# real-stanford/semantic-abstraction

Measured on AMD Instinct MI355X. Metric: scenes/sec (relevancy+3D-UNet infer), 480x480x16-label x128^3, higher is better.
Workload: dtype f16 (MFMA operands, fp32 accumulate; UNet hi/lo-split = fp32-equivalent); 1 GPU; end-to-end relevancy->fusion->OVSSC per scene: 480x480 RGB-D, 16 labels, ViT-B/16, 'ours' saliency config (2448 tile forwards), 128^3 voxels, 80000 input points; scene-sharded; arch=ViT-B/16, unet_precision=exact, tile_chunk_streams=1, scenes_per_gpu=26, parallelism=scene-shard x1, mode=throughput

## Files before the change

include/semabs.h:

```cpp
#ifndef SEMABS_H
#define SEMABS_H
#include <stdint.h>
#ifdef __cplusplus
extern "C" {
#endif

#define SEMABS_OK 0
#define SEMABS_EINVAL (-1)
#define SEMABS_EHIP (-2)

const char* semabs_last_error(void);
int semabs_abi_version(void);
int semabs_stream_create_cumask(const unsigned int* mask, int n_words, void** stream);
int semabs_stream_destroy(void* stream);
int semabs_stream_cu_count(void* stream, int* cus);

int semabs_fill_u32(void* p, long long nbytes, unsigned int value, void* stream);
int semabs_replicate(const void* src, void* dst, long long nbytes, int reps, void* stream);
int semabs_copy2d(const void* src, long long src_pitch_bytes, void* dst, long long dst_pitch_bytes, long long width_bytes, long long rows, void* stream);
int semabs_poison_empty(const long long* n_in, float* logits, long long n_logits, int* labels, long long n_labels, void* stream);
int semabs_device_info(char* name , int name_len, int* cu_count , long long* hbm_bytes );


int semabs_pointcloud(const float* depth, int H, int W, const double* params, int has_pose, float* xyz,
// ... 84 lines not shown

int semabs_point_mlp(const float* xyz, const float* feat, const float* w1, const float* b1, const float* w2, const float* b2,
                     const float* w3, const float* b3, float* out, int P, long N, int hidden, int cout, void* stream);
int semabs_point_mlp_fma(const float* xyz, const float* feat, const float* w1, const float* b1, const float* w2, const float* b2,
                         const float* w3, const float* b3, float* out, int P, long N, int hidden, int cout, void* stream);
int semabs_scatter_mean(const long long* flat, const float* feat, int* head, int* next, void* vol, int P, long N, int C,
                        long nvox, int vol_f32, void* stream);
int semabs_scatter_mean_stats(const long long* flat, const float* feat, int* head, int* next, void* vol, int P, long N, int C,
                              long nvox, int vol_f32, double* out_sums, void* stream);
int semabs_scatter_mean_sparse(const long long* flat, const float* feat, int* head, int* next, void* vol, unsigned int* occ, int P, long N, int C, long nvox,
                               int vol_f32, double* out_sums, void* stream);
int semabs_gn_stats(const void* x, double* sums, int B, long nvox, int C, int G, int x_f32, void* stream);
int semabs_gn_finalize(const double* sums, const float* gamma, const float* beta, float* scale, float* shift, int B, int C,
                       int G, long nvox, float eps, void* stream);
int semabs_conv3d(const void* x, const void* w_hi, const void* w_lo, void* y, const float* gn_scale, const float* gn_shift,
                  const float* bias, const void* resid, int B, int D0, int D1, int D2, int Cin, int Cout, int ksize, int relu,
                  int act_f32, void* stream);
int semabs_conv3d_stats(const void* x, const void* w_hi, const void* w_lo, void* y, const float* gn_scale, const float* gn_shift,
                        const float* bias, const void* resid, int B, int D0, int D1, int D2, int Cin, int Cout, int ksize, int relu,
                        int act_f32, double* out_sums, int out_groups, void* stream);
int semabs_conv3d_sparse_stats(const void* x, const unsigned int* occ, const void* w_hi, const void* w_lo, void* y, const float* gn_scale, const float* gn_shift,
                               const float* bias, const void* resid, int B, int D0, int D1, int D2, int Cin, int Cout, int ksize, int relu, int act_f32,
                               double* out_sums, int out_groups, void* stream);
int semabs_convtranspose3d(const void* x, const void* w_hi, const void* w_lo, const long* class_off , void* y,
                           const float* bias, const void* skip, int B, int D0, int D1, int D2, int Cin, int Cout, int act_f32,
                           void* stream);
int semabs_convtranspose3d_stats(const void* x, const void* w_hi, const void* w_lo, const long* class_off, void* y, const float* bias,
                                 const void* skip, int B, int D0, int D1, int D2, int Cin, int Cout, int act_f32, double* out_sums,
                                 int out_groups, void* stream);
int semabs_maxpool3d(const void* x, void* y, int B, int D0, int D1, int D2, int C, int act_f32, void* stream);
int semabs_decoder(const void* vol, const float* query, const float* off3, const float* sc3, const int* shape3, const float* w1,
                   const float* b1, const float* w2, const float* b2, int concat_xyz, int P, long M, long q_stride_p, int vol_f32,
                   float* out, const int* qgrid3, const float* final_w, const float* final_b, void* stream);

int semabs_vool_head(const void* vol_t, const void* vol_r, const float* query, const float* params, const float* rel,
                     const float* off3, const float* sc3, const int* shape3, float temperature, int P, long M, int vol_f32,
                     float* out, void* stream);


int semabs_lamb_step(const long long* chunks, int n_chunks, const long long* ptrs, int n_tensors, double lr, double beta1,
                     double beta2, double eps, double weight_decay, int adam, double* norms, float* stats, void* stream);


int semabs_conv3d_gather(const void* x, const void* w_hi, const void* w_lo, void* y, const float* in_scale, const float* in_shift, int B,
                         int I0, int I1, int I2, int M0, int M1, int M2, int in_stride, int Cin, int Cout, int ntaps, const signed char* taps,
                         int act_f32, void* stream);
// ... 83 lines not shown
```

semantic-abstraction_amd/_lib.py:

```python
from __future__ import annotations

import ctypes as C
import os

import torch

_HERE = os.path.dirname(os.path.abspath(__file__))
LIB_PATH = os.path.join(_HERE, "lib", "libsemabs_hip.so")
if os.environ.get("SEMABS_LIB_PATH"):
    LIB_PATH = os.environ["SEMABS_LIB_PATH"]
elif os.environ.get("SEMABS_TUNE_LIB") == "1":
    LIB_PATH = os.path.join(_HERE, "lib", "libsemabs_hip_tune.so")

_lib = None

P = C.c_void_p
I = C.c_int
L = C.c_long
F = C.c_float
D = C.c_double

SIGNATURES = {
    "semabs_abi_version": [],
    "semabs_stream_create_cumask": [P, I, P],
# ... 35 lines not shown
    "semabs_rows_gather": [P, P, L, I, L, L, P],
    "semabs_eot_rows_gather": [P, P, P, I, I, I, P],
    "semabs_quickgelu": [P, P, L, I, P],
    "semabs_quickgelu_grad": [P, P, L, P],
    "semabs_logit_grad": [P, P, I, I, I, P, P, P, I, P],
    "semabs_ln_bwd": [P, P, P, P, P, P, L, I, I, L, F, I, P],
    "semabs_gelu_bwd": [P, P, P, L, I, I, I, P],
    "semabs_rollout": [P, P, P, P, P, I, I, I, I, I, L, L, P],
    "semabs_gather_text": [P, P, P, P, I, I, I, P],
    "semabs_attention_bwd": [P, P, P, P, P, P, P, P, P, I, I, I, I, I, I, P],
    "semabs_seq_rescale": [P, P, P, L, L, P],
    "semabs_rollout_step": [P, P, L, P],
    "semabs_text_finish": [P, P, I, I, I, P],
    "semabs_point_mlp": [P, P, P, P, P, P, P, P, P, I, L, I, I, P],
    "semabs_point_mlp_fma": [P, P, P, P, P, P, P, P, P, I, L, I, I, P],
    "semabs_scatter_mean": [P, P, P, P, P, I, L, I, L, I, P],
    "semabs_scatter_mean_stats": [P, P, P, P, P, I, L, I, L, I, P, P],
    "semabs_scatter_mean_sparse": [P, P, P, P, P, P, I, L, I, L, I, P, P],
    "semabs_gn_stats": [P, P, I, L, I, I, I, P],
    "semabs_gn_finalize": [P, P, P, P, P, I, I, I, L, F, P],
    "semabs_conv3d": [P, P, P, P, P, P, P, P, I, I, I, I, I, I, I, I, I, P],
    "semabs_conv3d_stats": [P, P, P, P, P, P, P, P, I, I, I, I, I, I, I, I, I, P, I, P],
    "semabs_conv3d_sparse_stats": [P, P, P, P, P, P, P, P, P, I, I, I, I, I, I, I, I, I, P, I, P],
    "semabs_convtranspose3d": [P, P, P, C.POINTER(C.c_long), P, P, P, I, I, I, I, I, I, I, P],
    "semabs_convtranspose3d_stats": [P, P, P, C.POINTER(C.c_long), P, P, P, I, I, I, I, I, I, I, P, I, P],
    "semabs_maxpool3d": [P, P, I, I, I, I, I, I, P],
    "semabs_vool_head": [P, P, P, P, P, C.POINTER(F), C.POINTER(F), C.POINTER(I), F, I, L, I, P, P],
    "semabs_lamb_step": [P, I, P, I, D, D, D, D, D, I, P, P, P],
    "semabs_decoder": [P, P, C.POINTER(F), C.POINTER(F), C.POINTER(I), P, P, P, P, I, I, L, L, I, P, C.POINTER(I), P, P, P],
    "semabs_conv3d_gather": [P, P, P, P, P, P, I, I, I, I, I, I, I, I, I, I, I, C.c_char_p, I, P],
    "semabs_wgrad": [P, P, P, P, P, I, I, I, I, I, I, I, I, I, I, I, C.c_char_p, I, P],
    "semabs_wgrad_mfma": [P, P, P, P, P, P, P, I, I, I, I, I, I, I, I, I, I, I, C.c_char_p, I, P, L, P],
    "semabs_wgrad_conv3": [P, P, P, P, P, P, I, I, I, I, I, I, I, P, L, P],
    "semabs_wgrad_conv3_supported": [I, I, I, I, I, L, C.POINTER(I)],
    "semabs_conv3d_gnbwd_supported": [I, I, I, I, I, I, I, I, C.POINTER(I)],
    "semabs_conv3d_gnbwd": [P, P, P, P, P, P, P, P, P, P, I, P, I, P, I, I, I, I, I, I, I, P],
    "semabs_wgrad_conv3_gn_supported": [I, I, I, I, I, I, L, C.POINTER(I)],
    "semabs_wgrad_conv3_gn": [P, P, P, P, I, P, P, P, P, P, P, I, I, I, I, I, I, P, L, P],
    "semabs_chan_reduce": [P, P, P, P, P, I, L, I, I, P],
    "semabs_gn_meanrstd": [P, P, P, I, I, L, F, P],
    "semabs_gn_bwd_coef": [P, P, P, P, P, P, P, I, I, I, L, P],
    "semabs_gn_bwd_apply": [P, P, P, P, P, P, P, P, P, P, I, L, I, I, P],
    "semabs_ew": [P, P, P, L, I, F, P, P],
    "semabs_ew_scaled": [P, P, P, P, L, I, F, P, P],
    "semabs_grad_scale": [P, L, P, P, I, P, P, I, P],
    "semabs_maxpool3d_bwd": [P, P, P, I, I, I, I, I, P],
# ... 116 lines not shown
```

semantic-abstraction_amd/csrc/unet.hip:

```cpp
#include "semabs_common.h"

__device__ __forceinline__ int xcd_remap(int vb, int nb) {
    const int q = nb >> 3, r = nb & 7, x = vb & 7, k = vb >> 3;
    return (x < r ? x * (q + 1) : r * (q + 1) + (x - r) * q) + k;
}
__device__ __forceinline__ int xcd_persistent_tile(int vb, int G, int it, int total) {
    if (G & 7) { const long t = (long)it * G + vb; return t < total ? (int)t : -1; }
    const int x = vb & 7, j = vb >> 3, g8 = G >> 3;
    const int q = total >> 3, r = total & 7;
    const int lo = x < r ? x * (q + 1) : r * (q + 1) + (x - r) * q, cnt = q + (x < r ? 1 : 0);
    const long o = (long)it * g8 + j;
    return o < cnt ? lo + (int)o : -1;
}


template <int HID, int COUT>
__global__ __launch_bounds__(256, 2) void k_point_mlp(const float* __restrict__ xyz, const float* __restrict__ feat,
                                                   const float* __restrict__ w1, const float* __restrict__ b1,
                                                   const float* __restrict__ w2, const float* __restrict__ b2,
                                                   const float* __restrict__ w3, const float* __restrict__ b3,
                                                   float* __restrict__ out, int P, long N) {
    extern __shared__ __attribute__((aligned(16))) char smem[];
    float* sw2 = reinterpret_cast<float*>(smem);
    float* sw3 = sw2 + HID * HID;
// ... 384 lines not shown
#define CONV16_ABL(c) false
#endif
struct ConvArgs {
    const void* x; void* y; const f16* w_hi; const f16* w_lo;
    const float* gn_scale; const float* gn_shift; const float* bias; const void* resid;
    int B, I0, I1, I2;
    int O0, O1, O2;
    int M0, M1, M2;
    int os, op0, op1, op2;
    int Cin, Cout, Kp;
    int ntaps; int relu;
    int is;
    int ksplit;
    signed char td0[28], td1[28], td2[28];
    double* stats;
    int ablate;
    long long* trace;
    const f16* wp_hi; const f16* wp_lo;
    int ncls; long cls_off[8];
    const float* gnb_coef = nullptr; const float* gnb_mean = nullptr; const float* gnb_rstd = nullptr; int gnb_G = 0, gnb_relu = 0;
    unsigned int* gnb_bits = nullptr;
    const unsigned int* occ = nullptr;
    const float* gnb_add = nullptr;
};

template <bool F32>
__device__ __forceinline__ void load8(const void* base, long idx, float (&v)[8]) {
    if (F32) {
        const float4* p = reinterpret_cast<const float4*>(reinterpret_cast<const float*>(base) + idx);
        float4 a = p[0], b = p[1];
        v[0] = a.x; v[1] = a.y; v[2] = a.z; v[3] = a.w; v[4] = b.x; v[5] = b.y; v[6] = b.z; v[7] = b.w;
    } else {
        f16x8 h = *reinterpret_cast<const f16x8*>(reinterpret_cast<const f16*>(base) + idx);
#pragma unroll
        for (int j = 0; j < 8; ++j) v[j] = (float)h[j];
    }
}

template <int NW, bool F32, bool CIN16, bool LDSW = false, bool CLS = false>
__global__ __launch_bounds__(256) void k_conv(ConvArgs a) {
    const int ccls = CLS ? (int)blockIdx.z : 0;
    const int cp0 = CLS ? ccls >> 2 : 0, cp1 = CLS ? (ccls >> 1) & 1 : 0, cp2 = CLS ? ccls & 1 : 0;
    const int k_ntaps = CLS ? (cp0 + 1) * (cp1 + 1) * (cp2 + 1) : a.ntaps;
    const int k_Kp = CLS ? k_ntaps * a.Cin : a.Kp;
    const int k_op0 = CLS ? cp0 : a.op0, k_op1 = CLS ? cp1 : a.op1, k_op2 = CLS ? cp2 : a.op2;
    const long k_woff = CLS ? a.cls_off[ccls] : 0;
// ... 185 lines not shown
#pragma unroll
                for (int j = 0; j < 4; ++j) o[j] = o[j] > 0.f ? o[j] : 0.01f * o[j];
            }
            if (F32) {
                *reinterpret_cast<float4*>(reinterpret_cast<float*>(a.y) + oidx) = make_float4(o[0], o[1], o[2], o[3]);
            } else {
                f16x4 h; h[0] = (f16)o[0]; h[1] = (f16)o[1]; h[2] = (f16)o[2]; h[3] = (f16)o[3];
                *reinterpret_cast<f16x4*>(reinterpret_cast<f16*>(a.y) + oidx) = h;
            }
        }
    }
}

#define C16_T1 8
#define C16_T2 16
#define C16_H1 (C16_T1 + 2)
#define C16_H2 (C16_T2 + 2)

__device__ __forceinline__ void conv_absmax_commit(unsigned int* bits, float m) {
#pragma unroll
    for (int o = 1; o < 64; o <<= 1) m = fmaxf(m, __shfl_xor(m, o, 64));
    if ((threadIdx.x & 63) == 0) atomicMax(bits, __float_as_uint(m));
}
template <bool F32, int C16_T0, bool GNB = false, bool SPARSE = false>
__global__ __launch_bounds__(512) void k_conv16_lds(ConvArgs a) {
    constexpr int C16_H0 = C16_T0 + 2, C16_HALO = C16_H0 * C16_H1 * C16_H2;
    constexpr int PLANE = (C16_HALO * 8 + 127) / 128 * 128;
    constexpr int BUF_EL = PLANE * 2 * (F32 ? 2 : 1);
    extern __shared__ __attribute__((aligned(16))) char smem[];
    const int tid = threadIdx.x, lane = tid & 63;
    const int wid = __builtin_amdgcn_readfirstlane(tid >> 6);
    const int vl = lane & 15, kg = lane >> 4;
    const int n2 = a.I2 / C16_T2, n1 = a.I1 / C16_T1, n0 = a.I0 / C16_T0;
    const int per_vol = n0 * n1 * n2, total = a.B * per_vol;
    const bool has_gn = a.gn_scale != nullptr;
    const bool producer = wid >= 4;
    const int ptid = tid - 256;
    float* const s_gnb = reinterpret_cast<float*>(smem + (size_t)BUF_EL * 2 * 2);
    if (GNB) {
        for (int e = tid; e < a.B * 16; e += 512) {
            const int b = e >> 4, c = e & 15, g = c / (16 / a.gnb_G);
            const float mu = a.gnb_mean[b * a.gnb_G + g], rs = a.gnb_rstd[b * a.gnb_G + g];
            const float* k = a.gnb_coef + (long)e * 3;
            s_gnb[b * 48 + c] = k[0]; s_gnb[b * 48 + 16 + c] = -rs * k[2]; s_gnb[b * 48 + 32 + c] = mu * rs * k[2] - k[1];
        }
    }
    float amax = 0.f;

    auto produce = [&](int brick, int buf) {
        const int b = brick / per_vol; int t = brick - b * per_vol;
        const int t2 = t % n2; t /= n2;
        const int t1 = t % n1; const int t0 = t / n1;
        const int z0 = t0 * C16_T0, y0 = t1 * C16_T1, x0 = t2 * C16_T2;
        f16* s_hi = reinterpret_cast<f16*>(smem) + buf * BUF_EL;
        f16* s_lo = s_hi + PLANE * 2;
        const int hsel = (ptid >> 3) & 1;
        const int vsub = (ptid & 7) + ((ptid >> 4) << 3);
        float gs[8], gh[8];
        if (has_gn) {
            const float4* ps = reinterpret_cast<const float4*>(a.gn_scale + b * 16 + hsel * 8);
            const float4* pt = reinterpret_cast<const float4*>(a.gn_shift + b * 16 + hsel * 8);
            const float4 s0 = ps[0], s1 = ps[1], h0 = pt[0], h1 = pt[1];
            gs[0] = s0.x; gs[1] = s0.y; gs[2] = s0.z; gs[3] = s0.w; gs[4] = s1.x; gs[5] = s1.y; gs[6] = s1.z; gs[7] = s1.w;
            gh[0] = h0.x; gh[1] = h0.y; gh[2] = h0.z; gh[3] = h0.w; gh[4] = h1.x; gh[5] = h1.y; gh[6] = h1.z; gh[7] = h1.w;
        } else {
#pragma unroll
            for (int j = 0; j < 8; ++j) { gs[j] = 1.f; gh[j] = 0.f; }
        }
        constexpr int NT = (C16_HALO + 127) / 128;
// ... 69 lines not shown
                if (F32) wl[dy][st] = *reinterpret_cast<const f16x8*>(a.w_lo + widx);
            }
    };
    const int half = kg & 1, tsel = kg >> 1;
    f32x4 bias4 = f32x4{0.f, 0.f, 0.f, 0.f};
    if (a.bias) bias4 = *reinterpret_cast<const f32x4*>(a.bias + 4 * kg);
    const float relu_floor = a.relu ? 0.f : -__builtin_inff();
    double st[4] = {0.0, 0.0, 0.0, 0.0};
    int st_b = -1;
    auto flush_stats = [&]() {
        if (st_b >= 0) {
#pragma unroll
            for (int j = 0; j < 4; ++j) {
                double v = st[j];
#pragma unroll
                for (int m = 1; m < 16; m <<= 1) v += __shfl_xor(v, m, 64);
                if (vl == 0) atomicAdd(a.stats + ((long)st_b * 8 + 2 * kg + (j >> 1)) * 2 + (j & 1), v);
                st[j] = 0.0;
            }
        }
    };
    constexpr int ROWS_PER_WAVE = C16_T0 * 2;

    auto consume = [&](int brick, int buf) {
        const int b = brick / per_vol; int t = brick - b * per_vol;
        const int t2 = t % n2; t /= n2;
        const int t1 = t % n1; const int t0 = t / n1;
        const int z0 = t0 * C16_T0, y0 = t1 * C16_T1, x0 = t2 * C16_T2;
        const f16* s_hi = reinterpret_cast<const f16*>(smem) + buf * BUF_EL;
        const f16* s_lo = s_hi + PLANE * 2;
        const size_t vol_off = (size_t)b * a.I0 * a.I1 * a.I2 * 16;
        if (a.stats && b != st_b) { flush_stats(); st_b = b; }
        constexpr int MR = 8;
        int tapoff[5];
#pragma unroll
        for (int st = 0; st < 5; ++st) {
            const int qa = 2 * st, qb = 2 * st + 1 < 9 ? 2 * st + 1 : 2 * st;
            const int q = tsel ? qb : qa;
            tapoff[st] = ((q / 3) * C16_H1 * C16_H2 + (q % 3)) * 8;
        }
#pragma unroll 1
        for (int pr = 0; pr < ROWS_PER_WAVE / MR; ++pr) {
            const int zl = (wid * ROWS_PER_WAVE + pr * MR) >> 3;
            const int fbase = half * PLANE + (zl * C16_H1 * C16_H2 + vl) * 8;
            f32x4 acc[MR];
#pragma unroll
            for (int mi = 0; mi < MR; ++mi) acc[mi] = f32x4{0.f, 0.f, 0.f, 0.f};
            unsigned ooff[MR];
            f32x4 res[MR];
#pragma unroll
            for (int mi = 0; mi < MR; ++mi) {
                ooff[mi] = (unsigned)((((z0 + zl) * a.I1 + (y0 + mi)) * a.I2 + (x0 + vl)) * 16 + 4 * kg);
                res[mi] = f32x4{0.f, 0.f, 0.f, 0.f};
            }
            if (a.resid) {
// ... 24 lines not shown
                    const int i = st * 10 + ri, slot = i % 3, rho = RHO[ri];
                    bool first = true;
#pragma unroll
                    for (int kind = 0; kind < (F32 ? 3 : 1); ++kind) {
#pragma unroll
                        for (int dy = 0; dy < 3; ++dy) {
                            const int r = rho - dy;
                            if (r < 0 || r >= MR) continue;
                            acc[r] = __builtin_amdgcn_mfma_f32_16x16x32_f16(kind == 1 ? wl[dy][st] : wh[dy][st], kind == 2 ? xl[slot] : xh[slot], acc[r], 0, 0, 0);
                            if (first) {
                                first = false;
                                if (i + 2 < 50) request(i + 2, (i + 2) % 3);
                                __builtin_amdgcn_sched_barrier(0);
                            }
                        }
                    }
                    __builtin_amdgcn_sched_barrier(0);
                }
            }
#ifdef SEMABS_TUNING
            if (a.ablate == 4) { if (acc[0][0] != 1234.5f) continue; }
#endif
            float ps[4] = {0.f, 0.f, 0.f, 0.f};
            f32x4 cA, cB, cC;
            f32x4 ad[MR];
            if (GNB && a.gnb_add) {
                ad[0] = *reinterpret_cast<const f32x4*>(a.gnb_add + vol_off + ooff[0]);
                ad[1] = *reinterpret_cast<const f32x4*>(a.gnb_add + vol_off + ooff[1]);
            }
            if (GNB) {
                cA = *reinterpret_cast<const f32x4*>(s_gnb + b * 48 + 4 * kg); cB = *reinterpret_cast<const f32x4*>(s_gnb + b * 48 + 16 + 4 * kg);
                cC = *reinterpret_cast<const f32x4*>(s_gnb + b * 48 + 32 + 4 * kg);
            }
#pragma unroll
            for (int mi = 0; mi < MR; ++mi) {
                float o[4];
                if (GNB) {
                    if (a.gnb_add && mi + 2 < MR) { ad[mi + 2] = *reinterpret_cast<const f32x4*>(a.gnb_add + vol_off + ooff[mi + 2]); __builtin_amdgcn_sched_barrier(0); }
#pragma unroll
                    for (int e = 0; e < 4; ++e) {
                        o[e] = acc[mi][e] * cA[e] + (res[mi][e] * cB[e] + cC[e]);
                        if (a.gnb_add) o[e] += ad[mi][e];
                        if (a.gnb_relu) o[e] = res[mi][e] > 0.f ? o[e] : 0.f;
                        amax = fmaxf(amax, fabsf(o[e]));
                    }
                } else {
#pragma unroll
                for (int e = 0; e < 4; ++e) o[e] = fmaxf(acc[mi][e] + bias4[e] + res[mi][e], relu_floor);
                }
                if (!F32) {
#pragma unroll
                    for (int e = 0; e < 4; ++e) o[e] = (float)(f16)o[e];
                }
                ps[0] += o[0] + o[1]; ps[1] += o[0] * o[0] + o[1] * o[1];
                ps[2] += o[2] + o[3]; ps[3] += o[2] * o[2] + o[3] * o[3];
                if (F32) {
                    *reinterpret_cast<float4*>(reinterpret_cast<float*>(a.y) + vol_off + ooff[mi]) = make_float4(o[0], o[1], o[2], o[3]);
                } else {
                    f16x4 h; h[0] = (f16)o[0]; h[1] = (f16)o[1]; h[2] = (f16)o[2]; h[3] = (f16)o[3];
                    *reinterpret_cast<f16x4*>(reinterpret_cast<f16*>(a.y) + vol_off + ooff[mi]) = h;
                }
            }
            if (a.stats) {
#pragma unroll
                for (int j = 0; j < 4; ++j) st[j] += (double)ps[j];
            }
        }
    };

    auto lds_barrier = [&]() { asm volatile("s_waitcnt lgkmcnt(0)\n\ts_barrier" ::: "memory"); };
    auto brick_of = [&](int it) { return xcd_persistent_tile((int)blockIdx.x, (int)gridDim.x, it, total); };
    if (producer) {
        int it = 0, brick = brick_of(0);
        if (brick >= 0) produce(brick, 0);
        lds_barrier();
        int buf = 0;
        for (; brick >= 0; buf ^= 1) {
            const int next = brick_of(++it);
            if (next >= 0 && !CONV16_ABL(a.ablate == 2 || a.ablate >= 4)) produce(next, buf ^ 1);
            lds_barrier();
            brick = next;
        }
    } else {
        load_weights();
        lds_barrier();
        int buf = 0, it = 0;
        for (int brick = brick_of(0); brick >= 0; brick = brick_of(++it), buf ^= 1) {
            if (!CONV16_ABL(a.ablate == 1)) consume(brick, buf);
            lds_barrier();
        }
        if (a.stats) flush_stats();
        if (GNB && a.gnb_bits) conv_absmax_commit(a.gnb_bits, amax);
    }
}

#define SEMABS_CONV_GENERIC 256
#define SEMABS_CONV_PACKED 512
#ifdef SEMABS_TUNING
static int g_conv16_ablate = 0;
static long long* g_conv_trace = nullptr;
static int g_brick_persist = 0;
static int g_convt_no_line = 0;
extern "C" int semabs_conv_tune(int key, long long value) {
    if (key == 0) g_conv16_ablate = (int)value & 7;
    else if (key == 1) g_conv_trace = reinterpret_cast<long long*>(value);
    else if (key == 2) g_brick_persist = (int)value;
    else if (key == 3) g_convt_no_line = (int)value;
    return SEMABS_OK;
}
#endif

static int conv16_lds_launch(const ConvArgs& a_in, int f32, hipStream_t s) {
    ConvArgs a = a_in;
#ifdef SEMABS_TUNING
    a.ablate = g_conv16_ablate;
#endif
    if (f32) {
        constexpr int T0 = 4;
        const size_t lds = (size_t)(((T0 + 2) * C16_H1 * C16_H2 * 8 + 127) / 128 * 128) * 2 * 2 * 2 * 2;
        const long total = (long)a.B * (a.I0 / T0) * (a.I1 / C16_T1) * (a.I2 / C16_T2);
        long nb = semabs_stream_cus(s); if (nb > total) nb = total;
        if (a.gnb_coef) {
            static SemabsLdsAttr attrg;
            semabs_ensure_lds(&k_conv16_lds<true, T0, true>, (int)(lds + 32 * 192), attrg);
            hipLaunchKernelGGL((k_conv16_lds<true, T0, true>), dim3((unsigned)nb), dim3(512), lds + (size_t)a.B * 192, s, a);
            SEMABS_CHECK_LAUNCH();
            return SEMABS_OK;
        }
        if (a.occ) {
            static SemabsLdsAttr attrs;
            semabs_ensure_lds(&k_conv16_lds<true, T0, false, true>, (int)lds, attrs);
            hipLaunchKernelGGL((k_conv16_lds<true, T0, false, true>), dim3((unsigned)nb), dim3(512), lds, s, a);
            SEMABS_CHECK_LAUNCH();
            return SEMABS_OK;
        }
        static SemabsLdsAttr attr;
        semabs_ensure_lds(&k_conv16_lds<true, T0>, (int)lds, attr);
        hipLaunchKernelGGL((k_conv16_lds<true, T0>), dim3((unsigned)nb), dim3(512), lds, s, a);
    } else {
        constexpr int T0 = 8;
        const size_t lds = (size_t)(((T0 + 2) * C16_H1 * C16_H2 * 8 + 127) / 128 * 128) * 2 * 2 * 2;
        const long total = (long)a.B * (a.I0 / T0) * (a.I1 / C16_T1) * (a.I2 / C16_T2);
        long nb = semabs_stream_cus(s); if (nb > total) nb = total;
        if (a.occ) {
            static SemabsLdsAttr attrs;
            semabs_ensure_lds(&k_conv16_lds<false, T0, false, true>, (int)lds, attrs);
            hipLaunchKernelGGL((k_conv16_lds<false, T0, false, true>), dim3((unsigned)nb), dim3(512), lds, s, a);
            SEMABS_CHECK_LAUNCH();
            return SEMABS_OK;
        }
        static SemabsLdsAttr attr;
        semabs_ensure_lds(&k_conv16_lds<false, T0>, (int)lds, attr);
        hipLaunchKernelGGL((k_conv16_lds<false, T0>), dim3((unsigned)nb), dim3(512), lds, s, a);
    }
    SEMABS_CHECK_LAUNCH();
    return SEMABS_OK;
}

template <bool F32, int CW, int NB, bool ONE, bool PERSIST, int TX = 16, bool GNB = false>
__global__ __launch_bounds__(512) void k_conv_brick(ConvArgs a, int total) {
    constexpr int T0 = 4, H0 = T0 + 2, HX = TX + 2, HALO = H0 * C16_H1 * HX, NTHR = 512;
    constexpr int R = TX / 4;
    constexpr int CPV = CW / 8;
    constexpr int NSTEPS = CW == 32 ? 27 : 14;
    constexpr bool EARLY = false;
    extern __shared__ __attribute__((aligned(16))) char smem[];
    constexpr int PLANE = (HALO * 8 + 127) / 128 * 128;
    f16* s_hi = reinterpret_cast<f16*>(smem);
    f16* s_lo = s_hi + PLANE * CPV;
    const int tid = threadIdx.x, lane = tid & 63;
// ... 423 lines not shown
#define CONV_NW(F_, C_) { if (nw == 4) CONV_GO(4, F_, C_); else if (nw == 2) CONV_GO(2, F_, C_); else CONV_GO(1, F_, C_); }
    if (nw == 4 && !c16) {
        if (f32) hipLaunchKernelGGL((k_conv<4, true, false, true>), grid, block, 0, s, a);
        else hipLaunchKernelGGL((k_conv<4, false, false, true>), grid, block, 0, s, a);
    }
    else if (f32) { if (c16) CONV_NW(true, true) else CONV_NW(true, false) }
    else { if (c16) CONV_NW(false, true) else CONV_NW(false, false) }
#undef CONV_NW
#undef CONV_GO
    SEMABS_CHECK_LAUNCH();
    return SEMABS_OK;
}

static int conv_common_checks(const void* x, const void* w_hi, const void* w_lo, void* y, int Cin, int Cout, int f32) {
    SEMABS_REQUIRE(x && w_hi && y, "semabs conv: null pointer");
    SEMABS_REQUIRE(!f32 || w_lo, "semabs conv: exact (fp32) mode needs the lo half of the split weights");
    SEMABS_REQUIRE(Cin == 16 || Cin % 32 == 0, "semabs conv: Cin must be 16 or a multiple of 32");
    SEMABS_REQUIRE(Cout % 16 == 0 && (Cout < 64 || Cout % 64 == 0), "semabs conv: Cout must be 16, 32 or a multiple of 64");
    return SEMABS_OK;
}

static int conv3d_impl(const void* x, const void* w_hi, const void* w_lo, void* y, const float* gn_scale, const float* gn_shift,
                       const float* bias, const void* resid, int B, int D0, int D1, int D2, int Cin, int Cout, int ksize,
                       int relu, int act_flags, double* out_sums, int out_groups, void* stream, const unsigned int* occ = nullptr) {
    if (B == 0) return SEMABS_OK;
    const int act_f32 = act_flags & 1;
    const bool bricks = !(act_flags & SEMABS_CONV_GENERIC);
    int rc = conv_common_checks(x, w_hi, w_lo, y, Cin, Cout, act_f32);
    if (rc) return rc;
    SEMABS_REQUIRE(ksize == 1 || ksize == 3, "semabs_conv3d: kernel size must be 1 or 3");
    SEMABS_REQUIRE((gn_scale == nullptr) == (gn_shift == nullptr), "semabs_conv3d: gn_scale and gn_shift go together");
    ConvArgs a;
    a.x = x; a.y = y; a.w_hi = (const f16*)w_hi; a.w_lo = (const f16*)w_lo; a.gn_scale = gn_scale; a.gn_shift = gn_shift;
    a.bias = bias; a.resid = resid; a.B = B; a.I0 = D0; a.I1 = D1; a.I2 = D2; a.O0 = D0; a.O1 = D1; a.O2 = D2;
    a.M0 = D0; a.M1 = D1; a.M2 = D2; a.os = 1; a.is = 1; a.op0 = a.op1 = a.op2 = 0; a.Cin = Cin; a.Cout = Cout; a.relu = relu;
    a.ntaps = ksize * ksize * ksize;
    a.Kp = ((a.ntaps * Cin + 31) / 32) * 32;
    a.stats = nullptr; a.ablate = 0; a.trace = nullptr; a.wp_hi = nullptr; a.wp_lo = nullptr; a.ncls = 0;
    if (act_flags & SEMABS_CONV_PACKED) {
        a.wp_hi = a.w_hi + (long)Cout * a.Kp;
        if (w_lo) a.wp_lo = a.w_lo + (long)Cout * a.Kp;
    }
    int t = 0;
    for (int kd = 0; kd < ksize; ++kd)
        for (int kh = 0; kh < ksize; ++kh)
            for (int kw = 0; kw < ksize; ++kw, ++t) { a.td0[t] = kd - ksize / 2; a.td1[t] = kh - ksize / 2; a.td2[t] = kw - ksize / 2; }
    SEMABS_REQUIRE(relu == 0 || relu == 1 || (relu == 2 && ksize == 1), "semabs_conv3d: relu must be 0, 1, or 2 (LeakyReLU, ksize 1 only)");
    SEMABS_REQUIRE(!out_sums || (out_groups > 0 && Cout % out_groups == 0), "semabs_conv3d_stats: Cout must be a multiple of out_groups");
    bool fused = false;
    if (bricks && ksize == 3 && Cin == 16 && Cout == 16 && D0 % 8 == 0 && D1 % C16_T1 == 0 && D2 % C16_T2 == 0 && (long)D0 * D1 * D2 * 16 < (1L << 31)) {
        if (out_sums && out_groups == 8) { a.stats = out_sums; fused = true; }
        a.occ = occ;
        rc = conv16_lds_launch(a, act_f32, (hipStream_t)stream);
    } else if (occ) {
        semabs_set_error("semabs_conv3d_sparse_stats: the occupancy bitmap is read by the 16 -> 16 level-0 kernel only (D0 % 8, D1 % 8, D2 % 16 == 0)");
        return SEMABS_EINVAL;
    } else if (bricks && ksize == 3 && (Cout % 32 == 0 || (Cout == 16 && Cin % 32 == 0 && D2 % C16_T2 == 0)) && (Cin == 16 || Cin % 32 == 0) && relu != 2 &&
               D0 % 4 == 0 && D1 % C16_T1 == 0 && (D2 % C16_T2 == 0 || (D2 % 8 == 0 && Cin % 32 == 0))) {
        if (out_sums && out_groups == 8 && Cout >= 32) { a.stats = out_sums; fused = true; }
        rc = conv_brick_launch(a, act_f32, (hipStream_t)stream);
    } else {
        rc = conv_launch(a, act_f32, (hipStream_t)stream);
    }
    if (rc == SEMABS_OK && out_sums && !fused) rc = semabs_gn_stats(y, out_sums, B, (long)D0 * D1 * D2, Cout, out_groups, act_f32, stream);
    return rc;
}
extern "C" int semabs_conv3d(const void* x, const void* w_hi, const void* w_lo, void* y, const float* gn_scale, const float* gn_shift,
                             const float* bias, const void* resid, int B, int D0, int D1, int D2, int Cin, int Cout, int ksize,
                             int relu, int act_f32, void* stream) {
    return conv3d_impl(x, w_hi, w_lo, y, gn_scale, gn_shift, bias, resid, B, D0, D1, D2, Cin, Cout, ksize, relu, act_f32, nullptr, 0, stream);
}
extern "C" int semabs_conv3d_stats(const void* x, const void* w_hi, const void* w_lo, void* y, const float* gn_scale, const float* gn_shift,
                                   const float* bias, const void* resid, int B, int D0, int D1, int D2, int Cin, int Cout, int ksize,
                                   int relu, int act_f32, double* out_sums, int out_groups, void* stream) {
    SEMABS_REQUIRE(out_sums, "semabs_conv3d_stats: out_sums is null");
    return conv3d_impl(x, w_hi, w_lo, y, gn_scale, gn_shift, bias, resid, B, D0, D1, D2, Cin, Cout, ksize, relu, act_f32, out_sums, out_groups, stream);
}

extern "C" int semabs_conv3d_sparse_stats(const void* x, const unsigned int* occ, const void* w_hi, const void* w_lo, void* y, const float* gn_scale, const float* gn_shift,
                                          const float* bias, const void* resid, int B, int D0, int D1, int D2, int Cin, int Cout, int ksize,
                                          int relu, int act_f32, double* out_sums, int out_groups, void* stream) {
    SEMABS_REQUIRE(out_sums && occ, "semabs_conv3d_sparse_stats: out_sums / occ is null");
    SEMABS_REQUIRE(!(act_f32 & SEMABS_CONV_GENERIC), "semabs_conv3d_sparse_stats: the generic kernel reads the whole volume");
    return conv3d_impl(x, w_hi, w_lo, y, gn_scale, gn_shift, bias, resid, B, D0, D1, D2, Cin, Cout, ksize, relu, act_f32, out_sums, out_groups, stream, occ);
}

static int conv3d_gnbwd_route(int B, int D0, int D1, int D2, int Cin, int Cout, int G, bool have_add) {
    if (B <= 0 || G <= 0) return 0;
    if (B <= 32 && Cin == 16 && Cout == 16 && D0 % 8 == 0 && D1 % C16_T1 == 0 && D2 % C16_T2 == 0 && (long)D0 * D1 * D2 * 16 < (1L << 31) && 16 % G == 0) return 1;
    if (!have_add && Cin % 32 == 0 && Cout % 32 == 0 && Cout % G == 0 && (Cout / G) % 4 == 0 && D0 % 4 == 0 && D1 % C16_T1 == 0 && D2 % C16_T2 == 0) return 2;
    return 0;
}
extern "C" int semabs_conv3d_gnbwd_supported(int B, int D0, int D1, int D2, int Cin, int Cout, int G, int have_add1, int* ok) {
    SEMABS_REQUIRE(ok, "semabs_conv3d_gnbwd_supported: null pointer");
    *ok = conv3d_gnbwd_route(B, D0, D1, D2, Cin, Cout, G, have_add1 != 0) ? 1 : 0;
    return SEMABS_OK;
}
extern "C" int semabs_conv3d_gnbwd(const void* dZ, const void* w_hi, const void* w_lo, void* dX, const float* in_scale, const float* in_shift, const void* X,
                                   const float* mean, const float* rstd, const float* coef, int G, const float* add1, int relu_mask, unsigned int* absmax_bits,
                                   int B, int D0, int D1, int D2, int Cin, int Cout, int act_flags, void* stream) {
    if (B == 0) return SEMABS_OK;
    SEMABS_REQUIRE(dZ && w_hi && w_lo && dX && X && mean && rstd && coef, "semabs_conv3d_gnbwd: null pointer");
    const int route = conv3d_gnbwd_route(B, D0, D1, D2, Cin, Cout, G, add1 != nullptr);
    SEMABS_REQUIRE((act_flags & 1) && route, "semabs_conv3d_gnbwd: exact mode and a supported shape (see semabs_conv3d_gnbwd_supported)");
    SEMABS_REQUIRE((in_scale == nullptr) == (in_shift == nullptr), "semabs_conv3d_gnbwd: in_scale and in_shift go together");
    ConvArgs a;
    a.x = dZ; a.y = dX; a.w_hi = (const f16*)w_hi; a.w_lo = (const f16*)w_lo; a.gn_scale = in_scale; a.gn_shift = in_shift;
// ... 609 lines not shown
```

semantic-abstraction_amd/unet3d.py:

```python
from __future__ import annotations

import ctypes as C
from typing import Dict, List

import numpy as np
import torch

from . import _lib


def number_of_features_per_level(init_channel_number, num_levels):
    return [init_channel_number * 2 ** k for k in range(num_levels)]



def _pack_fragments(w: torch.Tensor) -> torch.Tensor:
    cout, kp = int(w.shape[0]), int(w.shape[1])
    assert cout % 16 == 0 and kp % 32 == 0
    return w.reshape(cout // 16, 16, kp // 32, 4, 8).permute(2, 0, 3, 1, 4).contiguous().reshape(-1)


def matrix_layout(m: torch.Tensor):
    rows, k = int(m.shape[0]), int(m.shape[1])
    kp = (k + 31) // 32 * 32
# ... 71 lines not shown
    def __init__(self, weight: torch.Tensor, bias, dev):
        flat, packed, offs = convT_class_layout(weight.float())
        self._set((*_split16(flat, dev), packed, offs), weight.shape, bias.float().to(dev).contiguous())

    def _set(self, fwd, wshape, bias):
        self.w_hi, self.w_lo, self.packed, offs = fwd
        self.class_off = (C.c_long * 8)(*offs)
        self.cin, self.cout = int(wshape[0]), int(wshape[1])
        self.bias = bias

    @classmethod
    def of(cls, name, fwd, bwd, wshape, bias):
        r = cls.__new__(cls)
        r.name, r.bwd = name, bwd
        r._set(fwd, wshape, bias)
        return r


class _Rec:
    __slots__ = ("name", "x", "y", "mean", "rstd", "scale", "shift")



def gn_conv(x, conv: _Conv, relu, zeros, f32, resid=None, gn=True, in_sums=None, out_groups=0, generic=False, occ=None, rec: _Rec | None = None):
    B, D0, D1, D2, Cc = x.shape
    nvox, dev, st = D0 * D1 * D2, x.device, _lib.stream()
    scale = shift = None
    if gn:
        G, sums = conv.groups, in_sums
        if sums is None:
            sums = zeros((B, G, 2), torch.float64)
            _lib.call("semabs_gn_stats", _lib.ptr(x), _lib.ptr(sums), B, nvox, Cc, G, f32, st)
        scale = torch.empty(B, Cc, dtype=torch.float32, device=dev)
        shift = torch.empty_like(scale)
        _lib.call("semabs_gn_finalize", _lib.ptr(sums), _lib.ptr(conv.gn_w), _lib.ptr(conv.gn_b), _lib.ptr(scale), _lib.ptr(shift),
                  B, Cc, G, nvox, 1e-5, st)
        if rec is not None:
            rec.mean = torch.empty(B, G, dtype=torch.float32, device=dev)
            rec.rstd = torch.empty_like(rec.mean)
            _lib.call("semabs_gn_meanrstd", _lib.ptr(sums), _lib.ptr(rec.mean), _lib.ptr(rec.rstd), B, G, nvox * (Cc // G), 1e-5, st)
    y = torch.empty(B, D0, D1, D2, conv.cout, dtype=torch.float32 if f32 else torch.float16, device=dev)
    if rec is not None:
        rec.name, rec.x, rec.y, rec.scale, rec.shift = conv.name, x, y, scale, shift
    args = (_lib.ptr(x), _lib.ptr(conv.w_hi), _lib.ptr(conv.w_lo), _lib.ptr(y), _lib.ptr(scale), _lib.ptr(shift),
            _lib.ptr(conv.bias), _lib.ptr(resid), B, D0, D1, D2, conv.cin, conv.cout, conv.k, int(relu), f32 | (256 if generic else 0) | conv.packed)
    if not out_groups:
        assert occ is None
        _lib.call("semabs_conv3d", *args, st)
        return y, None
    out_sums = zeros((B, out_groups, 2), torch.float64)
    if occ is not None:
        _lib.call("semabs_conv3d_sparse_stats", args[0], _lib.ptr(occ), *args[1:], _lib.ptr(out_sums), out_groups, st)
    else:
        _lib.call("semabs_conv3d_stats", *args, _lib.ptr(out_sums), out_groups, st)
    return y, out_sums


def res_block(x, convs, zeros, f32, in_sums=None, occ=None, tape=None):
    r1, r2, r3 = (None,) * 3 if tape is None else (_Rec(), _Rec(), _Rec())
    out1, s1 = gn_conv(x, convs[0], True, zeros, f32, in_sums=in_sums, out_groups=convs[1].groups, occ=occ, rec=r1)
    out2, s2 = gn_conv(out1, convs[1], True, zeros, f32, in_sums=s1, out_groups=convs[2].groups, rec=r2)
    y, _ = gn_conv(out2, convs[2], True, zeros, f32, resid=out1, in_sums=s2, rec=r3)
    if tape is not None:
        tape.append(("block", r1, r2, r3))
    return y


def maxpool(x, f32):
    B, D0, D1, D2, Cc = x.shape
    y = torch.empty(B, D0 // 2, D1 // 2, D2 // 2, Cc, dtype=x.dtype, device=x.device)
    _lib.call("semabs_maxpool3d", _lib.ptr(x), _lib.ptr(y), B, D0, D1, D2, Cc, f32, _lib.stream())
    return y


def up_conv(x, skip, ct: _ConvT, zeros, f32, out_groups=0, generic=False):
    B, D0, D1, D2, _ = x.shape
    assert tuple(skip.shape) == (B, 2 * D0, 2 * D1, 2 * D2, ct.cout)
    y = torch.empty_like(skip)
    args = (_lib.ptr(x), _lib.ptr(ct.w_hi), _lib.ptr(ct.w_lo), ct.class_off, _lib.ptr(y),
            _lib.ptr(ct.bias), _lib.ptr(skip), B, D0, D1, D2, ct.cin, ct.cout, f32 | (256 if generic else 0) | ct.packed)
    if not out_groups:
        _lib.call("semabs_convtranspose3d", *args, _lib.stream())
        return y, None
    sums = zeros((B, out_groups, 2), torch.float64)
    _lib.call("semabs_convtranspose3d_stats", *args, _lib.ptr(sums), out_groups, _lib.stream())
    return y, sums


def unet_forward(x, enc, dec, final: _Conv, zeros, f32, in_sums=None, occ=None, taps=None, skip_final=False, tape=None, rows_w=None):
    feats = []
    for i, convs in enumerate(enc):
        if i > 0:
            if tape is not None:
                tape.append(("pool", x, i - 1))
            x = maxpool(x, f32)
        x = res_block(x, convs, zeros, f32, in_sums=in_sums if i == 0 else None, occ=occ if i == 0 else None, tape=tape)
        if taps is not None:
            taps[f"enc{i}"] = x
        feats.insert(0, x)
    for i, (skip, (ct, convs)) in enumerate(zip(feats[1:], dec)):
        y, sums = up_conv(x, skip, ct, zeros, f32, out_groups=convs[0].groups)
        if tape is not None:
            tape.append(("up", ct.name, x, len(enc) - 2 - i))
        x = res_block(y, convs, zeros, f32, in_sums=sums, tape=tape)
        if taps is not None:
            taps[f"dec{i}"] = x
    if skip_final:
        return x
    if tape is not None:
        tape.append(("final", x))
    if rows_w is None:
        return gn_conv(x, final, False, zeros, f32, gn=False)[0]
    B, D0, D1, D2, _ = x.shape
    y = torch.empty(B, D0, D1, D2, final.cout, dtype=torch.float32, device=x.device)
    _lib.call("semabs_linear_rows", _lib.ptr(x), final.cin, _lib.ptr(rows_w), final.cin, 1, _lib.ptr(final.bias), _lib.ptr(y),
              B * D0 * D1 * D2, final.cin, final.cout, 0, 0.0, None, None, None, None, None, None, _lib.stream())
    return y


# ... 110 lines not shown
```

Before: 8.723 scenes/s.

## Fuse 2x2x2 maxpool and next-level GroupNorm stats into encoder conv epilogue

Adds a pooling variant of the 16-channel LDS conv kernel. It computes the 2x2x2 max inside the epilogue using DPP lane swaps and an LDS staging area, writes the pooled volume, and accumulates the GroupNorm sums for the next encoder level. The aim is to remove the separate maxpool launch and its full re-read of the level output, and to feed the next res_block's first conv with precomputed stats. Shapes that do not fit the kernel fall back to separate maxpool and gn_stats calls inside the same entry point. The cost is extra LDS per block, which may lower occupancy, plus an extra join phase after each brick's barrier.

```diff
diff --git a/include/semabs.h b/include/semabs.h
--- a/include/semabs.h
+++ b/include/semabs.h
@@ -130,6 +130,9 @@
 int semabs_conv3d_sparse_stats(const void* x, const unsigned int* occ, const void* w_hi, const void* w_lo, void* y, const float* gn_scale, const float* gn_shift,
                                const float* bias, const void* resid, int B, int D0, int D1, int D2, int Cin, int Cout, int ksize, int relu, int act_f32,
                                double* out_sums, int out_groups, void* stream);
+int semabs_conv3d_pool_stats(const void* x, const void* w_hi, const void* w_lo, void* y, void* y_pool, const float* gn_scale, const float* gn_shift,
+                             const float* bias, const void* resid, int B, int D0, int D1, int D2, int Cin, int Cout, int ksize, int relu,
+                             int act_f32, double* pool_sums, int pool_groups, void* stream);
 int semabs_convtranspose3d(const void* x, const void* w_hi, const void* w_lo, const long* class_off , void* y,
                            const float* bias, const void* skip, int B, int D0, int D1, int D2, int Cin, int Cout, int act_f32,
                            void* stream);
diff --git a/semantic-abstraction_amd/_lib.py b/semantic-abstraction_amd/_lib.py
--- a/semantic-abstraction_amd/_lib.py
+++ b/semantic-abstraction_amd/_lib.py
@@ -81,6 +81,7 @@
     "semabs_conv3d": [P, P, P, P, P, P, P, P, I, I, I, I, I, I, I, I, I, P],
     "semabs_conv3d_stats": [P, P, P, P, P, P, P, P, I, I, I, I, I, I, I, I, I, P, I, P],
     "semabs_conv3d_sparse_stats": [P, P, P, P, P, P, P, P, P, I, I, I, I, I, I, I, I, I, P, I, P],
+    "semabs_conv3d_pool_stats": [P, P, P, P, P, P, P, P, P, I, I, I, I, I, I, I, I, I, P, I, P],
     "semabs_convtranspose3d": [P, P, P, C.POINTER(C.c_long), P, P, P, I, I, I, I, I, I, I, P],
     "semabs_convtranspose3d_stats": [P, P, P, C.POINTER(C.c_long), P, P, P, I, I, I, I, I, I, I, P, I, P],
     "semabs_maxpool3d": [P, P, I, I, I, I, I, I, P],
diff --git a/semantic-abstraction_amd/csrc/unet.hip b/semantic-abstraction_amd/csrc/unet.hip
--- a/semantic-abstraction_amd/csrc/unet.hip
+++ b/semantic-abstraction_amd/csrc/unet.hip
@@ -430,6 +430,7 @@
     unsigned int* gnb_bits = nullptr;
     const unsigned int* occ = nullptr;
     const float* gnb_add = nullptr;
+    void* y_pool = nullptr;
 };
 
 template <bool F32>
@@ -661,8 +662,9 @@
     for (int o = 1; o < 64; o <<= 1) m = fmaxf(m, __shfl_xor(m, o, 64));
     if ((threadIdx.x & 63) == 0) atomicMax(bits, __float_as_uint(m));
 }
-template <bool F32, int C16_T0, bool GNB = false, bool SPARSE = false>
+template <bool F32, int C16_T0, bool GNB = false, bool SPARSE = false, bool POOL = false>
 __global__ __launch_bounds__(512) void k_conv16_lds(ConvArgs a) {
+    static_assert(!(POOL && (GNB || SPARSE)), "the pooling epilogue is instantiated for the plain forward kernel only");
     constexpr int C16_H0 = C16_T0 + 2, C16_HALO = C16_H0 * C16_H1 * C16_H2;
     constexpr int PLANE = (C16_HALO * 8 + 127) / 128 * 128;
     constexpr int BUF_EL = PLANE * 2 * (F32 ? 2 : 1);
@@ -684,6 +686,7 @@
             s_gnb[b * 48 + c] = k[0]; s_gnb[b * 48 + 16 + c] = -rs * k[2]; s_gnb[b * 48 + 32 + c] = mu * rs * k[2] - k[1];
         }
     }
+    float* const s_pool = reinterpret_cast<float*>(smem + (size_t)BUF_EL * 2 * 2);
     float amax = 0.f;
 
     auto produce = [&](int brick, int buf) {
@@ -799,7 +802,7 @@
     };
     constexpr int ROWS_PER_WAVE = C16_T0 * 2;
 
-    auto consume = [&](int brick, int buf) {
+    auto consume = [&](int brick, int buf, [[maybe_unused]] int par) {
         const int b = brick / per_vol; int t = brick - b * per_vol;
         const int t2 = t % n2; t /= n2;
         const int t1 = t % n1; const int t0 = t / n1;
@@ -807,7 +810,7 @@
         const f16* s_hi = reinterpret_cast<const f16*>(smem) + buf * BUF_EL;
         const f16* s_lo = s_hi + PLANE * 2;
         const size_t vol_off = (size_t)b * a.I0 * a.I1 * a.I2 * 16;
-        if (a.stats && b != st_b) { flush_stats(); st_b = b; }
+        if (!POOL && a.stats && b != st_b) { flush_stats(); st_b = b; }
         constexpr int MR = 8;
         int tapoff[5];
 #pragma unroll
@@ -878,6 +881,7 @@
             if (a.ablate == 4) { if (acc[0][0] != 1234.5f) continue; }
 #endif
             float ps[4] = {0.f, 0.f, 0.f, 0.f};
+            [[maybe_unused]] float prow[4] = {0.f, 0.f, 0.f, 0.f};
             f32x4 cA, cB, cC;
             f32x4 ad[MR];
             if (GNB && a.gnb_add) {
@@ -910,6 +914,22 @@
                 }
                 ps[0] += o[0] + o[1]; ps[1] += o[0] * o[0] + o[1] * o[1];
                 ps[2] += o[2] + o[3]; ps[3] += o[2] * o[2] + o[3] * o[3];
+                if constexpr (POOL) {
+                    if (mi & 1) {
+                        int pl = lane;
+                        asm volatile("" : "+v"(pl));
+                        f32x4 m;
+#pragma unroll
+                        for (int e = 0; e < 4; ++e) {
+                            const float v = fmaxf(prow[e], o[e]);
+                            m[e] = fmaxf(v, __int_as_float(__builtin_amdgcn_update_dpp(0, __float_as_int(v), 0xB1, 0xF, 0xF, true)));
+                        }
+                        if (!(pl & 1)) *reinterpret_cast<f32x4*>(s_pool + (((par * C16_T0 + zl) * 4 + (mi >> 1)) * 8 + ((pl & 15) >> 1)) * 16 + 4 * (pl >> 4)) = m;
+                    } else {
+#pragma unroll
+                        for (int e = 0; e < 4; ++e) prow[e] = o[e];
+                    }
+                }
                 if (F32) {
                     *reinterpret_cast<float4*>(reinterpret_cast<float*>(a.y) + vol_off + ooff[mi]) = make_float4(o[0], o[1], o[2], o[3]);
                 } else {
@@ -917,7 +937,7 @@
                     *reinterpret_cast<f16x4*>(reinterpret_cast<f16*>(a.y) + vol_off + ooff[mi]) = h;
                 }
             }
-            if (a.stats) {
+            if (!POOL && a.stats) {
 #pragma unroll
                 for (int j = 0; j < 4; ++j) st[j] += (double)ps[j];
             }
@@ -940,12 +960,55 @@
     } else {
         load_weights();
         lds_barrier();
+        [[maybe_unused]] auto flush_pool_stats = [&]() {
+            if (st_b >= 0) {
+#pragma unroll
+                for (int j = 0; j < 4; ++j) {
+                    double v = st[j];
+#pragma unroll
+                    for (int m = 4; m < 64; m <<= 1) v += __shfl_xor(v, m, 64);
+                    if (lane < 4) atomicAdd(a.stats + ((long)st_b * 8 + 2 * lane + (j >> 1)) * 2 + (j & 1), v);
+                    st[j] = 0.0;
+                }
+            }
+        };
+        [[maybe_unused]] auto join_pool = [&](int brick, int par) {
+            const int b = brick / per_vol; int t = brick - b * per_vol;
+            const int t2 = t % n2; t /= n2;
+            const int t1 = t % n1; const int t0 = t / n1;
+            const int P1 = a.I1 >> 1, P2 = a.I2 >> 1;
+            int pl = lane;
+            asm volatile("" : "+v"(pl));
+#pragma unroll
+            for (int j = 0; j < C16_T0 / 4; ++j) {
+                const int c = wid * (C16_T0 / 4) + j, p = c >> 1, py = (c & 1) * 2 + (pl >> 5), px = (pl >> 2) & 7, ch = (pl & 3) * 4;
+                const float* s0 = s_pool + (((par * C16_T0 + 2 * p) * 4 + py) * 8 + px) * 16 + ch;
+                const f32x4 u = *reinterpret_cast<const f32x4*>(s0), v = *reinterpret_cast<const f32x4*>(s0 + 4 * 8 * 16);
+                const float m0 = fmaxf(u[0], v[0]), m1 = fmaxf(u[1], v[1]), m2 = fmaxf(u[2], v[2]), m3 = fmaxf(u[3], v[3]);
+                if (a.stats) {
+                    if (b != st_b) { flush_pool_stats(); st_b = b; }
+                    const double d0 = (double)m0, d1 = (double)m1, d2 = (double)m2, d3 = (double)m3;
+                    st[0] += d0 + d1; st[1] += d0 * d0 + d1 * d1;
+                    st[2] += d2 + d3; st[3] += d2 * d2 + d3 * d3;
+                }
+                const size_t oidx = (size_t)b * (a.I0 >> 1) * P1 * P2 * 16 +
+                                    (unsigned)((((t0 * (C16_T0 / 2) + p) * P1 + t1 * (C16_T1 / 2) + py) * P2 + t2 * (C16_T2 / 2) + px) * 16 + ch);
+                if (F32) {
+                    *reinterpret_cast<float4*>(reinterpret_cast<float*>(a.y_pool) + oidx) = make_float4(m0, m1, m2, m3);
+                } else {
+                    f16x4 h; h[0] = (f16)m0; h[1] = (f16)m1; h[2] = (f16)m2; h[3] = (f16)m3;
+                    *reinterpret_cast<f16x4*>(reinterpret_cast<f16*>(a.y_pool) + oidx) = h;
+                }
+            }
+        };
         int buf = 0, it = 0;
         for (int brick = brick_of(0); brick >= 0; brick = brick_of(++it), buf ^= 1) {
-            if (!CONV16_ABL(a.ablate == 1)) consume(brick, buf);
+            if (!CONV16_ABL(a.ablate == 1)) consume(brick, buf, it & 1);
             lds_barrier();
-        }
-        if (a.stats) flush_stats();
+            if constexpr (POOL) join_pool(brick, it & 1);
+        }
+        if (!POOL && a.stats) flush_stats();
+        if constexpr (POOL) { if (a.stats) flush_pool_stats(); }
         if (GNB && a.gnb_bits) conv_absmax_commit(a.gnb_bits, amax);
     }
 }
@@ -990,6 +1053,13 @@
             SEMABS_CHECK_LAUNCH();
             return SEMABS_OK;
         }
+        if (a.y_pool) {
+            static SemabsLdsAttr attrp;
+            semabs_ensure_lds(&k_conv16_lds<true, T0, false, false, true>, (int)(lds + 2 * T0 * 2048), attrp);
+            hipLaunchKernelGGL((k_conv16_lds<true, T0, false, false, true>), dim3((unsigned)nb), dim3(512), lds + 2 * T0 * 2048, s, a);
+            SEMABS_CHECK_LAUNCH();
+            return SEMABS_OK;
+        }
         static SemabsLdsAttr attr;
         semabs_ensure_lds(&k_conv16_lds<true, T0>, (int)lds, attr);
         hipLaunchKernelGGL((k_conv16_lds<true, T0>), dim3((unsigned)nb), dim3(512), lds, s, a);
@@ -1002,6 +1072,13 @@
             static SemabsLdsAttr attrs;
             semabs_ensure_lds(&k_conv16_lds<false, T0, false, true>, (int)lds, attrs);
             hipLaunchKernelGGL((k_conv16_lds<false, T0, false, true>), dim3((unsigned)nb), dim3(512), lds, s, a);
+            SEMABS_CHECK_LAUNCH();
+            return SEMABS_OK;
+        }
+        if (a.y_pool) {
+            static SemabsLdsAttr attrp;
+            semabs_ensure_lds(&k_conv16_lds<false, T0, false, false, true>, (int)(lds + 2 * T0 * 2048), attrp);
+            hipLaunchKernelGGL((k_conv16_lds<false, T0, false, false, true>), dim3((unsigned)nb), dim3(512), lds + 2 * T0 * 2048, s, a);
             SEMABS_CHECK_LAUNCH();
             return SEMABS_OK;
         }
@@ -1471,7 +1548,8 @@
 
 static int conv3d_impl(const void* x, const void* w_hi, const void* w_lo, void* y, const float* gn_scale, const float* gn_shift,
                        const float* bias, const void* resid, int B, int D0, int D1, int D2, int Cin, int Cout, int ksize,
-                       int relu, int act_flags, double* out_sums, int out_groups, void* stream, const unsigned int* occ = nullptr) {
+                       int relu, int act_flags, double* out_sums, int out_groups, void* stream, const unsigned int* occ = nullptr,
+                       void* y_pool = nullptr, double* pool_sums = nullptr, int pool_groups = 0, int* pooled = nullptr) {
     if (B == 0) return SEMABS_OK;
     const int act_f32 = act_flags & 1;
     const bool bricks = !(act_flags & SEMABS_CONV_GENERIC);
@@ -1500,6 +1578,10 @@
     if (bricks && ksize == 3 && Cin == 16 && Cout == 16 && D0 % 8 == 0 && D1 % C16_T1 == 0 && D2 % C16_T2 == 0 && (long)D0 * D1 * D2 * 16 < (1L << 31)) {
         if (out_sums && out_groups == 8) { a.stats = out_sums; fused = true; }
         a.occ = occ;
+        if (y_pool && !occ) {
+            a.y_pool = y_pool; *pooled = 1;
+            if (!out_sums && pool_groups == 8) { a.stats = pool_sums; *pooled = 2; }
+        }
         rc = conv16_lds_launch(a, act_f32, (hipStream_t)stream);
     } else if (occ) {
         semabs_set_error("semabs_conv3d_sparse_stats: the occupancy bitmap is read by the 16 -> 16 level-0 kernel only (D0 % 8, D1 % 8, D2 % 16 == 0)");
@@ -1532,6 +1614,21 @@
     SEMABS_REQUIRE(out_sums && occ, "semabs_conv3d_sparse_stats: out_sums / occ is null");
     SEMABS_REQUIRE(!(act_f32 & SEMABS_CONV_GENERIC), "semabs_conv3d_sparse_stats: the generic kernel reads the whole volume");
     return conv3d_impl(x, w_hi, w_lo, y, gn_scale, gn_shift, bias, resid, B, D0, D1, D2, Cin, Cout, ksize, relu, act_f32, out_sums, out_groups, stream, occ);
+}
+
+extern "C" int semabs_maxpool3d(const void* x, void* y, int B, int D0, int D1, int D2, int C, int act_f32, void* stream);
+extern "C" int semabs_conv3d_pool_stats(const void* x, const void* w_hi, const void* w_lo, void* y, void* y_pool, const float* gn_scale, const float* gn_shift,
+                                        const float* bias, const void* resid, int B, int D0, int D1, int D2, int Cin, int Cout, int ksize,
+                                        int relu, int act_f32, double* pool_sums, int pool_groups, void* stream) {
+    SEMABS_REQUIRE(y_pool && pool_sums, "semabs_conv3d_pool_stats: y_pool / pool_sums is null");
+    SEMABS_REQUIRE(D0 % 2 == 0 && D1 % 2 == 0 && D2 % 2 == 0 && Cout % 8 == 0, "semabs_conv3d_pool_stats: dims must be even, Cout % 8 == 0");
+    SEMABS_REQUIRE(pool_groups > 0 && Cout % pool_groups == 0, "semabs_conv3d_pool_stats: Cout must be a multiple of pool_groups");
+    int pooled = 0;
+    int rc = conv3d_impl(x, w_hi, w_lo, y, gn_scale, gn_shift, bias, resid, B, D0, D1, D2, Cin, Cout, ksize, relu, act_f32, nullptr, 0, stream, nullptr, y_pool,
+                         pool_sums, pool_groups, &pooled);
+    if (rc == SEMABS_OK && pooled < 1) rc = semabs_maxpool3d(y, y_pool, B, D0, D1, D2, Cout, act_f32 & 1, stream);
+    if (rc == SEMABS_OK && pooled < 2) rc = semabs_gn_stats(y_pool, pool_sums, B, (long)(D0 / 2) * (D1 / 2) * (D2 / 2), Cout, pool_groups, act_f32 & 1, stream);
+    return rc;
 }
 
 static int conv3d_gnbwd_route(int B, int D0, int D1, int D2, int Cin, int Cout, int G, bool have_add) {
diff --git a/semantic-abstraction_amd/unet3d.py b/semantic-abstraction_amd/unet3d.py
--- a/semantic-abstraction_amd/unet3d.py
+++ b/semantic-abstraction_amd/unet3d.py
@@ -117,7 +117,8 @@
 
 
 
-def gn_conv(x, conv: _Conv, relu, zeros, f32, resid=None, gn=True, in_sums=None, out_groups=0, generic=False, occ=None, rec: _Rec | None = None):
+def gn_conv(x, conv: _Conv, relu, zeros, f32, resid=None, gn=True, in_sums=None, out_groups=0, generic=False, occ=None, rec: _Rec | None = None,
+            pool_groups=0):
     B, D0, D1, D2, Cc = x.shape
     nvox, dev, st = D0 * D1 * D2, x.device, _lib.stream()
     scale = shift = None
@@ -139,6 +140,12 @@
         rec.name, rec.x, rec.y, rec.scale, rec.shift = conv.name, x, y, scale, shift
     args = (_lib.ptr(x), _lib.ptr(conv.w_hi), _lib.ptr(conv.w_lo), _lib.ptr(y), _lib.ptr(scale), _lib.ptr(shift),
             _lib.ptr(conv.bias), _lib.ptr(resid), B, D0, D1, D2, conv.cin, conv.cout, conv.k, int(relu), f32 | (256 if generic else 0) | conv.packed)
+    if pool_groups:
+        assert not out_groups and occ is None and rec is None
+        y_pool = torch.empty(B, D0 // 2, D1 // 2, D2 // 2, conv.cout, dtype=y.dtype, device=dev)
+        pool_sums = zeros((B, pool_groups, 2), torch.float64)
+        _lib.call("semabs_conv3d_pool_stats", *args[:4], _lib.ptr(y_pool), *args[4:], _lib.ptr(pool_sums), pool_groups, st)
+        return y, (y_pool, pool_sums)
     if not out_groups:
         assert occ is None
         _lib.call("semabs_conv3d", *args, st)
@@ -151,14 +158,17 @@
     return y, out_sums
 
 
-def res_block(x, convs, zeros, f32, in_sums=None, occ=None, tape=None):
+def res_block(x, convs, zeros, f32, in_sums=None, occ=None, tape=None, pool_groups=0):
     r1, r2, r3 = (None,) * 3 if tape is None else (_Rec(), _Rec(), _Rec())
     out1, s1 = gn_conv(x, convs[0], True, zeros, f32, in_sums=in_sums, out_groups=convs[1].groups, occ=occ, rec=r1)
     out2, s2 = gn_conv(out1, convs[1], True, zeros, f32, in_sums=s1, out_groups=convs[2].groups, rec=r2)
-    y, _ = gn_conv(out2, convs[2], True, zeros, f32, resid=out1, in_sums=s2, rec=r3)
+    y, pooled = gn_conv(out2, convs[2], True, zeros, f32, resid=out1, in_sums=s2, rec=r3, pool_groups=pool_groups)
     if tape is not None:
         tape.append(("block", r1, r2, r3))
-    return y
+    return (y, pooled) if pool_groups else y
+
+
+FUSE_POOL = True
 
 
 def maxpool(x, f32):
@@ -184,12 +194,19 @@
 
 def unet_forward(x, enc, dec, final: _Conv, zeros, f32, in_sums=None, occ=None, taps=None, skip_final=False, tape=None, rows_w=None):
     feats = []
+    pooled = None
     for i, convs in enumerate(enc):
+        sums = in_sums if i == 0 else None
         if i > 0:
-            if tape is not None:
-                tape.append(("pool", x, i - 1))
-            x = maxpool(x, f32)
-        x = res_block(x, convs, zeros, f32, in_sums=in_sums if i == 0 else None, occ=occ if i == 0 else None, tape=tape)
+            if pooled is not None:
+                x, sums = pooled
+            else:
+                if tape is not None:
+                    tape.append(("pool", x, i - 1))
+                x = maxpool(x, f32)
+        pg = enc[i + 1][0].groups if FUSE_POOL and tape is None and i + 1 < len(enc) else 0
+        x = res_block(x, convs, zeros, f32, in_sums=sums, occ=occ if i == 0 else None, tape=tape, pool_groups=pg)
+        x, pooled = x if pg else (x, None)
         if taps is not None:
             taps[f"enc{i}"] = x
         feats.insert(0, x)
```

After: 8.738 scenes/s, median of 2. No clear change (+0.2%).
